# ideafisher/ssUnet-GAN

Measured on AMD Instinct MI355X. Metric: train images/sec (512^2 tiles), higher is better.
Workload: dtype f32; 1 GPU; UNet_R_SS_v2 generator + SRGAN-style discriminator, one G+D step (train_seg_gan.py:182-233), 16 x 3x512x512 tiles per GPU, fp32, Adam lr 2e-5; global_batch=16, tile=512, parallelism=dp1, dead_d_param_grads_of_g_step=computed

## Files before the change

### include/ssunet_hip.h

```cpp
#ifndef SSUNET_HIP_H
#define SSUNET_HIP_H

#include <stdint.h>

#ifdef __cplusplus
extern "C" {
#endif

#define SSG_OK 0
#define SSG_EINVAL (-1)
#define SSG_EALIGN (-2)

#define SSG_ACT_NONE 0
#define SSG_ACT_RELU 1
#define SSG_ACT_LRELU 2
#define SSG_ACT_SWISH 3

#define SSG_MAX_TAPS 9

const char* ssg_last_error(void);
int ssg_abi_version(void);

typedef struct {
  const float* in1; const float* in2;
// ... 154 lines not shown
                        float* mean, float* invstd, float* scale, float* shift, void* stream);

typedef struct ssg_bn_fin {
  const float* weight; const float* bias;
  float eps, momentum; int var_mode;
  float* running_mean; float* running_var;
  float* mean; float* invstd; float* scale; float* shift;
} ssg_bn_fin;
int ssg_bn_stats_finalize_f32(const float* x, int64_t P, int C, int ld, const ssg_bn_fin* fin, void* ws, void* stream);
int ssg_bn_stats_finalize_bf16(const void* x, int64_t P, int C, int ld, const ssg_bn_fin* fin, void* ws, void* stream);
int ssg_bn_stats_from_partials_finalize_f32(const double* part, int rows, int C, double count, const ssg_bn_fin* fin, void* ws, void* stream);
int ssg_bn_apply_f32(const float* x, int64_t P, int C, int ld, const float* scale, const float* shift,
                     const float* res, int ldr, int act, float slope, float* y, int ldy, void* stream);
int ssg_bn_bwd_reduce_f32(const float* x, const float* y, const float* dy, int64_t P, int C,
                          int ldx, int ldy, int lddy, const float* mean, const float* invstd,
                          const float* scale, const float* shift,
                          int act, float slope, double* sums, int with_count, void* ws, void* stream);
int ssg_bn_bwd_apply_f32(const float* x, const float* y, const float* dy, int64_t P, int C,
                         int ldx, int ldy, int lddy, const float* mean, const float* invstd,
                         const float* weight, const float* scale, const float* shift,
                         const double* sums, double count, int act, float slope,
                         float* dx, int lddx, float* dres, int lddres,
                         float* dweight, float* dbias, void* stream);
int ssg_bn_frozen_bwd_f32(const float* x, const float* y, const float* dy, int64_t P, int C, int ldx, int ldy, int lddy,
                          const float* mean, const float* invstd, const float* scale, const float* shift, int act, float slope,
                          float* dx, int lddx, float* dres, int lddres, double* sums, void* ws, void* stream);
int ssg_bn_fold_bwd_f32(const float* dwf, const float* w, int Cout, int64_t K, const float* s, const float* mean,
                        const float* invstd, const double* sums_g, float* dw, float* dgamma, float* dbeta, void* stream);

int ssg_maxpool2x2_fwd_f32(const float* x, int N, int H, int W, int C, int ldx, float* y, int ldy, uint8_t* idx, void* stream);
int ssg_maxpool2x2_bwd_f32(const float* dy, int lddy, const uint8_t* idx, int N, int H, int W, int C, float* dx, int lddx, void* stream);
int ssg_maxpool2x2_bwd_add_f32(const float* dy, int lddy, const uint8_t* idx, const float* res, int ldr, int N, int H, int W, int C,
                               float* dx, int lddx, void* stream);
int ssg_maxunpool2x2_fwd_f32(const float* x, int ldx, const uint8_t* idx, int N, int OH, int OW, int C, float* y, int ldy, void* stream);
int ssg_maxunpool2x2_bwd_f32(const float* dy, int lddy, const uint8_t* idx, int N, int OH, int OW, int C, float* dx, int lddx, void* stream);
int ssg_upsample2x_bilinear_fwd_f32(const float* x, int N, int H, int W, int C, int ldx, float* y, int ldy, void* stream);
int ssg_upsample2x_bilinear_bwd_f32(const float* dy, int lddy, int N, int H, int W, int C, float* dx, int lddx, void* stream);
int ssg_upsample2x_nearest_fwd_f32(const float* x, int N, int H, int W, int C, int ldx, float* y, int ldy, void* stream);
int ssg_upsample2x_nearest_bwd_f32(const float* dy, int lddy, int N, int H, int W, int C, float* dx, int lddx, void* stream);
int ssg_adaptive_avgpool_flat_fwd_f32(const float* x, int N, int H, int W, int C, int ldx, int OHW, float* y, void* stream);
int ssg_adaptive_avgpool_flat_bwd_f32(const float* dy, int N, int H, int W, int C, int OHW, float* dx, int lddx, void* stream);

int ssg_spade_conv_modulate_ok(const ssg_conv_desc* d);
int ssg_spade_conv_modulate_f32(const ssg_conv_desc* d, const float* x, int ldx, float* gamma, int ldg, void* stream);
int ssg_spade_modulate_fwd_f32(const float* x, int ldx, const float* gb, int ldgb, int64_t P, int C, float* y, int ldy, void* stream);
int ssg_spade_modulate_bwd_f32(const float* x, int ldx, const float* gb, int ldgb, const float* dy, int lddy, int64_t P, int C,
// ... 97 lines not shown
```

### ssunet-gan_amd/_lib.py

```python
import ctypes as C
import os

import torch

_HERE = os.path.dirname(os.path.abspath(__file__))
LIB_PATH = os.environ.get('SSG_LIB_PATH') or os.path.join(_HERE, 'libssunet_hip.so')
MAX_TAPS = 9
ACT_NONE, ACT_RELU, ACT_LRELU, ACT_SWISH = 0, 1, 2, 3


class HipLibraryError(RuntimeError):
    pass


class ConvDesc(C.Structure):
    _fields_ = [
        ('in1', C.c_void_p), ('in2', C.c_void_p),
        ('C1', C.c_int), ('C2', C.c_int), ('ld1', C.c_int), ('ld2', C.c_int),
        ('N', C.c_int), ('H', C.c_int), ('W', C.c_int),
        ('w', C.c_void_p), ('Kp', C.c_int), ('kmode', C.c_int),
        ('bias', C.c_void_p),
        ('res', C.c_void_p), ('ldr', C.c_int),
        ('out', C.c_void_p), ('Cout', C.c_int), ('ldo', C.c_int),
        ('GH', C.c_int), ('GW', C.c_int), ('OH', C.c_int), ('OW', C.c_int),
# ... 80 lines not shown
    'ssg_conv2d_wgrad_bf16x2_ok': [C.POINTER(WgradDesc)],
    'ssg_conv2d_wgrad_bf16x2_kernel_id': [C.POINTER(WgradDesc)],
    'ssg_conv2d_wgrad_bf16x2_workspace_bytes': [C.POINTER(WgradDesc)],
    'ssg_conv2d_wgrad_bf16x2_f32': [C.POINTER(WgradDesc), _P],
    'ssg_conv2d_wgrad_bf16x1_s2_ok': [C.POINTER(WgradDesc)],
    'ssg_conv2d_wgrad_bf16x1_s2_kernel_id': [C.POINTER(WgradDesc)],
    'ssg_conv2d_wgrad_bf16x1_s2_workspace_bytes': [C.POINTER(WgradDesc)],
    'ssg_conv2d_wgrad_bf16x1_s2_f32': [C.POINTER(WgradDesc), _P],
    'ssg_bn_stats_from_partials_workspace_bytes': [_I, _I],
    'ssg_bn_stats_from_partials_f32': [_P, _I, _I, _P, _D, _P, _P],
    'ssg_conv2d_wgrad_kernel_id': [C.POINTER(WgradDesc)],
    'ssg_pack_weights_f32': [_P, _I, _I, _I, _I, _I, _I, C.POINTER(C.c_int), C.POINTER(C.c_int), _I, _I, _I, _P, _P],
    'ssg_pack_weights_scaled_f32': [_P, _I, _I, _I, _I, _I, _I, C.POINTER(C.c_int), C.POINTER(C.c_int), _I, _I, _I, _P, _P, _P],
    'ssg_conv2d_wgrad_workspace_bytes': [C.POINTER(WgradDesc)],
    'ssg_conv2d_wgrad_f32': [C.POINTER(WgradDesc), _P],
    'ssg_nchw_to_nhwc_f32': [_P, _I, _I, _I, _I, _P, _I, _P],
    'ssg_nhwc_to_nchw_f32': [_P, _I, _I, _I, _I, _I, _P, _P],
    'ssg_bn_workspace_bytes': [_L, _I],
    'ssg_bn_stats_f32': [_P, _L, _I, _I, _P, _I, _P, _P],
    'ssg_bn_finalize_f32': [_P, _D, _I, _P, _P, _F, _F, _I, _P, _P, _P, _P, _P, _P, _P],
    'ssg_bn_apply_f32': [_P, _L, _I, _I, _P, _P, _P, _I, _I, _F, _P, _I, _P],
    'ssg_bn_bwd_reduce_f32': [_P, _P, _P, _L, _I, _I, _I, _I, _P, _P, _P, _P, _I, _F, _P, _I, _P, _P],
    'ssg_bn_bwd_apply_f32': [_P, _P, _P, _L, _I, _I, _I, _I, _P, _P, _P, _P, _P, _P, _D, _I, _F, _P, _I, _P, _I, _P, _P, _P],
    'ssg_bn_frozen_bwd_f32': [_P, _P, _P, _L, _I, _I, _I, _I, _P, _P, _P, _P, _I, _F, _P, _I, _P, _I, _P, _P, _P],
    'ssg_bn_fold_bwd_f32': [_P, _P, _I, _L, _P, _P, _P, _P, _P, _P, _P, _P],
    'ssg_maxpool2x2_fwd_f32': [_P, _I, _I, _I, _I, _I, _P, _I, _P, _P],
    'ssg_maxpool2x2_bwd_f32': [_P, _I, _P, _I, _I, _I, _I, _P, _I, _P],
    'ssg_maxpool2x2_bwd_add_f32': [_P, _I, _P, _P, _I, _I, _I, _I, _I, _P, _I, _P],
    'ssg_maxunpool2x2_fwd_f32': [_P, _I, _P, _I, _I, _I, _I, _P, _I, _P],
    'ssg_maxunpool2x2_bwd_f32': [_P, _I, _P, _I, _I, _I, _I, _P, _I, _P],
    'ssg_upsample2x_bilinear_fwd_f32': [_P, _I, _I, _I, _I, _I, _P, _I, _P],
    'ssg_upsample2x_bilinear_bwd_f32': [_P, _I, _I, _I, _I, _I, _P, _I, _P],
    'ssg_upsample2x_nearest_fwd_f32': [_P, _I, _I, _I, _I, _I, _P, _I, _P],
    'ssg_upsample2x_nearest_bwd_f32': [_P, _I, _I, _I, _I, _I, _P, _I, _P],
    'ssg_adaptive_avgpool_flat_fwd_f32': [_P, _I, _I, _I, _I, _I, _I, _P, _P],
    'ssg_adaptive_avgpool_flat_bwd_f32': [_P, _I, _I, _I, _I, _I, _P, _I, _P],
    'ssg_spade_conv_modulate_ok': [C.POINTER(ConvDesc)],
    'ssg_spade_conv_modulate_f32': [C.POINTER(ConvDesc), _P, _I, _P, _I, _P],
    'ssg_spade_modulate_fwd_f32': [_P, _I, _P, _I, _L, _I, _P, _I, _P],
    'ssg_spade_modulate_bwd_f32': [_P, _I, _P, _I, _P, _I, _L, _I, _P, _I, _P, _I, _P],
    'ssg_spade_modulate_bwd_sums_f32': [_P, _I, _P, _I, _P, _I, _L, _I, _P, _I, _P, _I, _P, _P, _P],
    'ssg_act_bwd_f32': [_P, _I, _P, _I, _L, _I, _I, _F, _P, _I, _P],
    'ssg_add_f32': [_P, _P, _L, _P, _P],
    'ssg_copy_channels_f32': [_P, _I, _L, _I, _P, _I, _P],
    'ssg_nan_to_zero_f32': [_P, _L, _P, _P],
    'ssg_mask_zero_f32': [_P, _P, _L, _P, _P],
# ... 139 lines not shown
```

### ssunet-gan_amd/blocks.py

```python
import ctypes as C
import os

import torch

from . import ops
from ._lib import ACT_NONE, ACT_RELU, call, ptr, stream_ptr
from .ops import (_act_bwd, _bn_bwd_impl, _bn_fwd_impl, _channel_sum, _conv_dgrad_impl, _conv_fwd_impl, _conv_wgrad_impl,
                  _ld, new_nhwc, to_nhwc)


def _x_mode(stride):
    mode = ops.train_precision_mode()
    return mode if mode != 'fp32' and stride == 1 else False


class _BasicBlockFn(torch.autograd.Function):

    @staticmethod
    def forward(ctx, x1, x2, w1, g1, b1, rm1, rv1, w2, g2, b2, rm2, rv2, wsc, eps1, mom1, eps2, mom2, stride, var_mode, group):
        x1 = to_nhwc(x1)
        x2 = to_nhwc(x2) if x2 is not None else None
        ctx.x1m = x1m = _x_mode(stride)
        p3 = x1m or 'fp32'
        c1, part1 = _conv_fwd_impl(x1, x2, w1, None, stride, 1, ACT_NONE, 0.0, want_bn=True, precision=p3)
# ... 55 lines not shown
        dx1 = dx2 = None
        if stride != 1 and (need_x1 or need_x2):
            raise NotImplementedError('strided BasicBlock input gradient')
        if need_x1:
            part = _conv_dgrad_impl(g, wsc, 1, 0, h, w, 0, ca) if wsc is not None else g
            dx1 = _conv_dgrad_impl(dc1, w1, 1, 1, h, w, 0, ca, res=part, precision=p3)
        if need_x2:
            part = _conv_dgrad_impl(g, wsc, 1, 0, h, w, ca, ca + cb)
            dx2 = _conv_dgrad_impl(dc1, w1, 1, 1, h, w, ca, ca + cb, res=part, precision=p3)
        return (dx1, dx2, dw1, dg1, db1, None, None, dw2, dg2, db2, None, None, dwsc,
                None, None, None, None, None, None, None)


def basic_block(x1, x2, conv1, bn1, conv2, bn2, shortcut_conv, group=None):
    for bn in (bn1, bn2):
        if bn.track_running_stats and bn.num_batches_tracked is not None and not ops._synced(group):
            bn.num_batches_tracked.add_(1)
    var_mode = getattr(bn1, '_ssg_var_mode', 1 if group is not None else 0)
    return _BasicBlockFn.apply(x1, x2, conv1.weight, bn1.weight, bn1.bias, bn1.running_mean, bn1.running_var,
                               conv2.weight, bn2.weight, bn2.bias, bn2.running_mean, bn2.running_var,
                               shortcut_conv.weight if shortcut_conv is not None else None,
                               float(bn1.eps), float(bn1.momentum), float(bn2.eps), float(bn2.momentum),
                               int(conv1.stride[0]), var_mode, group)


def _fold_bwd(dwf, w, s, mean, invstd, sums_g, need_w, need_gb):
    o = w.shape[0]
    dw = torch.empty_like(dwf) if need_w else None
    dgb = torch.empty((2, o), dtype=torch.float32, device=w.device) if need_gb else None
    wc = w.detach().contiguous()
    call('ssg_bn_fold_bwd_f32', ptr(dwf), ptr(wc), o, wc.numel() // o, ptr(s), ptr(mean), ptr(invstd), ptr(sums_g), ptr(dw),
         ptr(dgb[0]) if need_gb else None, ptr(dgb[1]) if need_gb else None, stream_ptr())
    return dw, (dgb[0] if need_gb else None), (dgb[1] if need_gb else None)


class _FrozenBasicBlockFn(torch.autograd.Function):

    @staticmethod
    def forward(ctx, x1, x2, w1, g1, b1, w2, g2, b2, wsc, wf1, bf1, wf2, bf2, k1, k2, stride, record):
        x1 = to_nhwc(x1)
        x2 = to_nhwc(x2) if x2 is not None else None
        x1m = record and any(ctx.needs_input_grad) and _x_mode(stride)
        p3 = x1m or 'fp32'
        y1 = _conv_fwd_impl(x1, x2, wf1, bf1, stride, 1, ACT_RELU, 0.0, precision=p3)
        if wsc is not None:
            r = _conv_fwd_impl(x1, x2, wsc, None, stride, 0, ACT_NONE, 0.0)
# ... 233 lines not shown
```

### ssunet-gan_amd/csrc/bn.hip

```cpp
#include "common.h"

namespace {

constexpr int RED_BLOCK = 256;
constexpr int MAX_PARTS = 1024;

struct RedGeom { int TQ, PR, groups, parts; long long rows_per_part; };

__host__ RedGeom red_geom(long long P, int C, int Q = 1) {
  RedGeom g;
  const int CQ = (C + 4 * Q - 1) / (4 * Q);
  g.TQ = CQ >= 64 ? 64 : 1;
  if (CQ < 64) { while (g.TQ < CQ) g.TQ <<= 1; }
  g.PR = RED_BLOCK / g.TQ;
  g.groups = (CQ + g.TQ - 1) / g.TQ;
  long long parts = (P + (long long)g.PR * 8 - 1) / ((long long)g.PR * 8);
  if (parts > MAX_PARTS) parts = MAX_PARTS;
  if (parts < 1) parts = 1;
  g.rows_per_part = (P + parts - 1) / parts;
  g.parts = (int)((P + g.rows_per_part - 1) / g.rows_per_part);
  return g;
}

template <int MODE, typename T>
// ... 252 lines not shown
                                                       const T* __restrict__ res, int ldr, int act, float slope,
                                                       T* __restrict__ y, int ldy) {
  constexpr int Q = SsgQ<T>::value;
  const int CG = C / (4 * Q);
  const long long total = P * CG;
  SSG_CHUNK_LOOP(i, total) {
    const long long p = i / CG; const int c0 = 4 * Q * (int)(i - p * CG);
    f32x4 xv[Q], rv[Q], o[Q];
    ldq(x + p * ld + c0, xv);
    if (res) ldq(res + p * ldr + c0, rv);
#pragma unroll
    for (int q = 0; q < Q; ++q) {
      const f32x4 sc = *(const f32x4*)(scale + c0 + 4 * q), sh = *(const f32x4*)(shift + c0 + 4 * q);
      f32x4 v = xv[q] * sc + sh;
      if (res) v += rv[q];
#pragma unroll
      for (int e = 0; e < 4; ++e) v[e] = ssg_act(v[e], act, slope);
      o[q] = v;
    }
    stq(y + p * ldy + c0, o);
  }
}

template <typename T>
__global__ __launch_bounds__(256) void bn_bwd_apply_kernel(
    const T* __restrict__ x, const T* __restrict__ y, const T* __restrict__ dy, long long P, int C, int ldx,
    int ldy, int lddy, const float* __restrict__ mean, const float* __restrict__ invstd, const float* __restrict__ weight,
    const float* __restrict__ scale, const float* __restrict__ shift,
    const double* __restrict__ sums, double count_arg, int act, float slope, T* __restrict__ dx, int lddx,
    T* __restrict__ dres, int lddres, float* __restrict__ dweight, float* __restrict__ dbias) {
  const double count = count_arg > 0 ? count_arg : sums[2 * C];
  if (blockIdx.x == 0) {
    for (int c = threadIdx.x; c < C; c += 256) {
      if (dweight) dweight[c] = (float)sums[C + c];
      if (dbias) dbias[c] = (float)sums[c];
    }
  }
  typedef typename SsgAcc<T>::type acc_t;
  extern __shared__ double kc_raw[];
  acc_t* kc = (acc_t*)kc_raw;
  acc_t* k_mean = kc; acc_t* k_is = kc + C; acc_t* k_ws = kc + 2 * C; acc_t* k_m1 = kc + 3 * C; acc_t* k_m2 = kc + 4 * C;
  for (int c = threadIdx.x; c < C; c += 256) {
    const double is = (double)invstd[c];
    k_mean[c] = (acc_t)mean[c]; k_is[c] = (acc_t)is; k_ws[c] = (acc_t)((weight ? (double)weight[c] : 1.0) * is);
    k_m1[c] = (acc_t)(sums[c] / count); k_m2[c] = (acc_t)(sums[C + c] / count);
  }
  __syncthreads();
  constexpr int Q = SsgQ<T>::value;
  const int CG = C / (4 * Q);
  const long long totalg = P * CG;
  SSG_CHUNK_LOOP(i, totalg) {
    const long long p = i / CG; const int c0 = 4 * Q * (int)(i - p * CG);
    f32x4 gq[Q], xq[Q], yq[Q], oq[Q];
    ldq(dy + p * lddy + c0, gq);
    ldq(x + p * ldx + c0, xq);
    const bool use_y = act != SSG_ACT_NONE && act != SSG_ACT_SWISH && y;
    if (use_y) ldq(y + p * ldy + c0, yq);
#pragma unroll
    for (int q = 0; q < Q; ++q) {
      const int cb = c0 + 4 * q;
      f32x4 g = gq[q];
      const f32x4 xv = xq[q];
      if (act == SSG_ACT_SWISH) {
        const f32x4 z = xv * *(const f32x4*)(scale + cb) + *(const f32x4*)(shift + cb);
#pragma unroll
        for (int e = 0; e < 4; ++e) g[e] *= ssg_swish_grad(z[e]);
      } else if (act != SSG_ACT_NONE) {
        const f32x4 yv = use_y ? yq[q] : xv * *(const f32x4*)(scale + cb) + *(const f32x4*)(shift + cb);
#pragma unroll
        for (int e = 0; e < 4; ++e) if (!(yv[e] > 0.f)) g[e] *= (act == SSG_ACT_RELU ? 0.f : slope);
      }
      gq[q] = g;
      if (dx) {
        f32x4 o;
#pragma unroll
        for (int e = 0; e < 4; ++e) {
          const int c = cb + e;
          const acc_t xh = ((acc_t)xv[e] - k_mean[c]) * k_is[c];
          o[e] = (float)(k_ws[c] * ((acc_t)g[e] - k_m1[c] - xh * k_m2[c]));
        }
        oq[q] = o;
      }
    }
    if (dres) stq(dres + p * lddres + c0, gq);
    if (dx) stq(dx + p * lddx + c0, oq);
  }
}

int elem_grid(long long total) { return ssg_elem_grid(total, 4); }

template <int MODE, typename T>
int run_reduce(const T* x, const T* y, const T* dy, long long P, int C, int ldx, int ldy, int lddy,
               const float* scale, const float* shift,
               const float* mean, const float* invstd, int act, float slope, double* sums, float* fsum, void* ws,
               hipStream_t st, double count_out = 0.0, BnFin fin = BnFin{}, double fin_count = 0.0) {
  constexpr int Q = SsgQ<T>::value;
  const RedGeom g = red_geom(P, C, Q);
  const int C4 = 4 * Q * ((C + 4 * Q - 1) / (4 * Q));
  double* part = (double*)ws;
  hipLaunchKernelGGL((col_reduce_kernel<MODE, T>), dim3((unsigned)g.parts, (unsigned)g.groups), dim3(RED_BLOCK), 0, st, x, y, dy,
                     P, C, ldx, ldy, lddy, mean, invstd, scale, shift, act, slope, g.TQ, g.PR, g.rows_per_part, part, (T*)nullptr, 0, (T*)nullptr, 0);
  SSG_LAUNCH_CHECK();
  hipLaunchKernelGGL(col_reduce_final_kernel, dim3((unsigned)((C + 31) / 32)), dim3(32 * FIN_LANES), 0, st, part, g.parts, C, C4, sums, fsum, count_out, fin, fin_count);
  SSG_LAUNCH_CHECK();
  return SSG_OK;
}

}
// ... 26 lines not shown
  SSG_REQUIRE(!(act == SSG_ACT_SWISH && res), SSG_EINVAL, "bn_apply: swish with a residual is not supported (its backward needs the pre-activation)");
  hipLaunchKernelGGL(bn_apply_kernel<T>, dim3((unsigned)elem_grid(P * (C / (4 * SsgQ<T>::value)))), dim3(256), 0, (hipStream_t)stream, x, (long long)P, C, ld,
                     scale, shift, res, ldr, act, slope, y, ldy);
  SSG_LAUNCH_CHECK();
  return SSG_OK;
}

template <typename T>
int bn_bwd_reduce_impl(const T* x, const T* y, const T* dy, int64_t P, int C, int ldx, int ldy, int lddy, const float* mean,
                       const float* invstd, const float* scale, const float* shift, int act, float slope, double* sums, int with_count,
                       void* ws, void* stream) {
  SSG_REQUIRE(x && dy && mean && invstd && sums && ws && P > 0 && C > 0, SSG_EINVAL, "bn_bwd_reduce: bad args");
  SSG_REQUIRE(act == SSG_ACT_NONE || (y && act != SSG_ACT_SWISH) || (scale && shift), SSG_EINVAL,
              "bn_bwd_reduce: activation gradient needs y (ReLU family only) or (scale, shift)");
  SSG_REQUIRE(C % (4 * SsgQ<T>::value) == 0 && ldx % (4 * SsgQ<T>::value) == 0 && lddy % (4 * SsgQ<T>::value) == 0 && ssg_aligned16(x) && ssg_aligned16(dy),
              SSG_EALIGN, "bn_bwd_reduce: C / ld must be multiples of 4 (fp32) or 8 (bf16), rows 16-byte aligned");
  return run_reduce<1, T>(x, y, dy, P, C, ldx, ldy, lddy, scale, shift, mean, invstd, act, slope, sums, nullptr, ws, (hipStream_t)stream,
                          with_count ? (double)P : 0.0);
}

template <typename T>
int bn_bwd_apply_impl(const T* x, const T* y, const T* dy, int64_t P, int C, int ldx, int ldy, int lddy, const float* mean,
                      const float* invstd, const float* weight, const float* scale, const float* shift, const double* sums, double count,
                      int act, float slope, T* dx, int lddx, T* dres, int lddres, float* dweight, float* dbias, void* stream) {
  SSG_REQUIRE(x && dy && mean && invstd && sums && P > 0 && C > 0, SSG_EINVAL, "bn_bwd_apply: bad args");
  SSG_REQUIRE(act == SSG_ACT_NONE || (y && act != SSG_ACT_SWISH) || (scale && shift), SSG_EINVAL,
              "bn_bwd_apply: activation gradient needs y (ReLU family only) or (scale, shift)");
  constexpr int G = 4 * SsgQ<T>::value;
  SSG_REQUIRE(C % G == 0 && ldx % G == 0 && lddy % G == 0 && (!y || ldy % G == 0) && (!dx || lddx % G == 0) && (!dres || lddres % G == 0) &&
                  ssg_aligned16(x) && ssg_aligned16(dy) && (!dx || ssg_aligned16(dx)), SSG_EALIGN,
              "bn_bwd_apply: C/ld must be multiples of 4 (fp32) or 8 (bf16), rows 16-byte aligned");
  SSG_REQUIRE(C <= 4096, SSG_EINVAL, "bn_bwd_apply: C > 4096");
  if ((size_t)5 * C * sizeof(double) > 48 * 1024) {
    hipError_t e = hipFuncSetAttribute((const void*)bn_bwd_apply_kernel<T>, hipFuncAttributeMaxDynamicSharedMemorySize, 5 * C * (int)sizeof(double));
    if (e != hipSuccess) { ssg_set_error("bn_bwd_apply: LDS attribute: %s", hipGetErrorString(e)); return (int)e; }
  }
  hipLaunchKernelGGL(bn_bwd_apply_kernel<T>, dim3((unsigned)elem_grid(P * (C / (4 * SsgQ<T>::value)))), dim3(256), (size_t)5 * C * sizeof(double), (hipStream_t)stream, x, y, dy,
                     (long long)P, C, ldx, ldy, lddy, mean, invstd, weight, scale, shift, sums, count, act, slope, dx, lddx, dres, lddres,
                     dweight, dbias);
  SSG_LAUNCH_CHECK();
  return SSG_OK;
}

}

extern "C" int ssg_bn_stats_f32(const float* x, int64_t P, int C, int ld, double* sums, int with_count, void* ws, void* stream) {
  return bn_stats_impl<float>(x, P, C, ld, sums, with_count, ws, stream);
}
extern "C" int ssg_bn_stats_bf16(const void* x, int64_t P, int C, int ld, double* sums, int with_count, void* ws, void* stream) {
  return bn_stats_impl<ssg_bf16>((const ssg_bf16*)x, P, C, ld, sums, with_count, ws, stream);
}

namespace {
constexpr int FOLD_Z = 64;
__global__ __launch_bounds__(256) void bnpart_fold_kernel(const double* __restrict__ part, int rows, int C, int rows_per_z,
                                                          double* __restrict__ out ) {
  __shared__ double red[2][8][32];
  const int cl = threadIdx.x & 31, rl = threadIdx.x >> 5;
  const int c = blockIdx.x * 32 + cl;
  const int r0 = blockIdx.y * rows_per_z;
  int r1 = r0 + rows_per_z; if (r1 > rows) r1 = rows;
  double a1 = 0, a2 = 0;
// ... 92 lines not shown
                                 const void* res, int ldr, int act, float slope, void* y, int ldy, void* stream) {
  return bn_apply_impl<ssg_bf16>((const ssg_bf16*)x, P, C, ld, scale, shift, (const ssg_bf16*)res, ldr, act, slope, (ssg_bf16*)y, ldy, stream);
}

extern "C" int ssg_bn_bwd_reduce_f32(const float* x, const float* y, const float* dy, int64_t P, int C, int ldx, int ldy,
                                     int lddy, const float* mean, const float* invstd, const float* scale, const float* shift,
                                     int act, float slope, double* sums, int with_count, void* ws, void* stream) {
  return bn_bwd_reduce_impl<float>(x, y, dy, P, C, ldx, ldy, lddy, mean, invstd, scale, shift, act, slope, sums, with_count, ws, stream);
}
extern "C" int ssg_bn_bwd_reduce_bf16(const void* x, const void* y, const void* dy, int64_t P, int C, int ldx, int ldy,
                                      int lddy, const float* mean, const float* invstd, const float* scale, const float* shift,
                                      int act, float slope, double* sums, int with_count, void* ws, void* stream) {
  return bn_bwd_reduce_impl<ssg_bf16>((const ssg_bf16*)x, (const ssg_bf16*)y, (const ssg_bf16*)dy, P, C, ldx, ldy, lddy, mean, invstd, scale, shift,
                                      act, slope, sums, with_count, ws, stream);
}

extern "C" int ssg_bn_bwd_apply_f32(const float* x, const float* y, const float* dy, int64_t P, int C, int ldx, int ldy,
                                    int lddy, const float* mean, const float* invstd, const float* weight,
                                    const float* scale, const float* shift, const double* sums,
                                    double count, int act, float slope, float* dx, int lddx, float* dres, int lddres,
                                    float* dweight, float* dbias, void* stream) {
  return bn_bwd_apply_impl<float>(x, y, dy, P, C, ldx, ldy, lddy, mean, invstd, weight, scale, shift, sums, count, act, slope, dx, lddx, dres,
                                  lddres, dweight, dbias, stream);
}
extern "C" int ssg_bn_bwd_apply_bf16(const void* x, const void* y, const void* dy, int64_t P, int C, int ldx, int ldy,
                                     int lddy, const float* mean, const float* invstd, const float* weight,
                                     const float* scale, const float* shift, const double* sums,
                                     double count, int act, float slope, void* dx, int lddx, void* dres, int lddres,
                                     float* dweight, float* dbias, void* stream) {
  return bn_bwd_apply_impl<ssg_bf16>((const ssg_bf16*)x, (const ssg_bf16*)y, (const ssg_bf16*)dy, P, C, ldx, ldy, lddy, mean, invstd, weight, scale,
                                     shift, sums, count, act, slope, (ssg_bf16*)dx, lddx, (ssg_bf16*)dres, lddres, dweight, dbias, stream);
}

extern "C" int ssg_spade_modulate_bwd_sums_f32(const float* x, int ldx, const float* gb, int ldgb, const float* dy, int lddy, int64_t P,
                                               int C, float* dx, int lddx, float* dgb, int lddgb, double* sums, void* ws, void* stream) {
  SSG_REQUIRE(x && gb && dy && dx && dgb && sums && ws && P > 0 && C > 0 && C % 4 == 0 && ldgb >= C && lddgb >= 2 * C, SSG_EINVAL,
              "modulate_bwd_sums: bad args");
  const RedGeom g = red_geom(P, C);
  double* part = (double*)ws;
  hipStream_t st = (hipStream_t)stream;
  hipLaunchKernelGGL(modulate_bwd_sums_kernel, dim3((unsigned)g.parts, (unsigned)g.groups), dim3(RED_BLOCK), 0, st, x, ldx, gb, ldgb, dy, lddy,
                     (long long)P, C, dx, lddx, dgb, lddgb, g.TQ, g.PR, g.rows_per_part, part);
  SSG_LAUNCH_CHECK();
  hipLaunchKernelGGL(col_reduce_final_kernel, dim3((unsigned)((C + 31) / 32)), dim3(32 * FIN_LANES), 0, st, part, g.parts, C, C, sums, nullptr, 0.0, BnFin{}, 0.0);
  SSG_LAUNCH_CHECK();
  return SSG_OK;
// ... 88 lines not shown
```

### ssunet-gan_amd/models_seg_gan.py

```python
import os

import torch
import torch.nn as nn

from . import archs, ops
from ._lib import ACT_LRELU, ACT_NONE
from .spectral_norm import SpectralNorm


def remove_prefix(state_dict, prefix):
    f = lambda x: x.split(prefix, 1)[-1] if x.startswith(prefix) else x
    return {f(key): value for key, value in state_dict.items()}


class ConvolutionalBlock(nn.Module):

    def __init__(self, in_channels, out_channels, kernel_size, stride=1, batch_norm=False, activation=None):
        super().__init__()
        if activation is not None:
            activation = activation.lower()
            assert activation in {'prelu', 'leakyrelu', 'tanh'}
        layers = [nn.Conv2d(in_channels=in_channels, out_channels=out_channels, kernel_size=kernel_size, stride=stride,
                            padding=kernel_size // 2)]
        if batch_norm is True:
            layers.append(nn.BatchNorm2d(num_features=out_channels))
        if activation == 'prelu':
            layers.append(nn.PReLU())
        elif activation == 'leakyrelu':
# ... 10 lines not shown
        for hook in conv._forward_pre_hooks.values():
            if isinstance(hook, SpectralNorm) and hook.name == 'weight' and hook.dim == 0 and conv.weight_orig.is_cuda:
                sn = hook
            else:
                hook(conv, (input,))
        if self._act not in (None, 'leakyrelu'):
            raise NotImplementedError('ConvolutionalBlock activation %r has no HIP path (only the discriminator\'s '
                                      'LeakyReLU flavour is on the hot path)' % self._act)
        act = ACT_LRELU if self._act == 'leakyrelu' else ACT_NONE
        slope = self.conv_block[-1].negative_slope if act == ACT_LRELU else 0.0
        if sn is not None:
            def run(a, sl):
                return ops.conv2d_sn(input, conv.weight_orig, conv.weight_u, conv.weight_v, conv.bias, conv.stride[0], conv.padding[0],
                                     act=a, slope=sl, n_power_iterations=sn.n_power_iterations if conv.training else 0, eps=sn.eps)
        else:
            precision, wgrad_s2 = ops.train_precision_mode(), ops.train_wgrad_s2_mode()

            def run(a, sl, bn_stats=False):
                return ops.conv2d(input, conv.weight, conv.bias, conv.stride[0], conv.padding[0], act=a, slope=sl, bn_stats=bn_stats,
                                  precision=precision, wgrad_s2=wgrad_s2)
        if not self._bn:
            return run(act, slope)
        bn = self.conv_block[1]
        part = None
        if sn is None and bn.training:
            y, part = run(ACT_NONE, 0.0, bn_stats=True)
        else:
            y = run(ACT_NONE, 0.0)
        return ops.batch_norm_act(y, bn, act=act, slope=slope, group=getattr(bn, '_ssg_sync_group', None), stats_part=part)


class Generator(nn.Module):

    def __init__(self, config):
        super().__init__()
        if config['arch'] not in archs.__all__:
            raise NotImplementedError('arch %r is not built in ssunet-gan_amd (available: %s)' % (config['arch'], archs.__all__))
        self.net = archs.__dict__[config['arch']](config['num_classes'], config['input_channels'], config['deep_supervision'])

    def initialize_with_srresnet(self, model_folder, config):
        model_dict = torch.load(os.path.join(model_folder, '%s/model.pth' % config['name']), map_location='cpu')
        if 'state_dict' in model_dict.keys():
            model_dict = remove_prefix(model_dict['state_dict'], 'module.')
        else:
            model_dict = remove_prefix(model_dict, 'module.')
        missing, unexpected = self.net.load_state_dict(model_dict, strict=False)
        if missing or unexpected:
            raise RuntimeError('checkpoint key mismatch: missing %s unexpected %s' % (missing[:5], unexpected[:5]))
        print("\nLoaded weights from pre-trained SS-UNet-R.\n")

    def forward(self, lr_imgs):
        return self.net(lr_imgs)
# ... 26 lines not shown
```

### ssunet-gan_amd/ops.py

```python
import ctypes as C
import math

import torch
import torch.distributed as dist

from . import _lib
from ._lib import ACT_LRELU, ACT_NONE, ACT_RELU, ACT_SWISH, ConvDesc, WgradDesc, call, ptr, stream_ptr

__all__ = ['conv2d', 'batch_norm_act', 'max_pool2x2', 'max_pool2x2_skip', 'max_unpool2x2', 'upsample2x_bilinear', 'upsample2x_nearest',
           'spade_modulate', 'adaptive_avgpool_flat', 'linear', 'seg_loss', 'bce_with_logits_const', 'nan_to_zero_',
           'to_nhwc', 'new_nhwc', 'bump_weight_epoch', 'dwconv2d', 'swish', 'sigmoid', 'gaussian', 'mul', 'global_avgpool',
           'channel_scale', 'spectral_norm_weight', 'conv2d_sn']


def pad4(c):
    return (c + 3) // 4 * 4


def new_nhwc(n, c, h, w, device, ld=None, zero=False):
    ld = pad4(c) if ld is None else ld
    buf = (torch.zeros if zero else torch.empty)(n * h * w * ld, device=device, dtype=torch.float32)
    return torch.empty(0, device=device, dtype=torch.float32).set_(
        buf.untyped_storage(), 0, (n, c, h, w), (h * w * ld, 1, w * ld, ld))

# ... 505 lines not shown
        ctx.set_materialize_grads(False)
        x1 = to_nhwc(x1)
        x2 = to_nhwc(x2) if x2 is not None else None
        res = to_nhwc(res) if res is not None else None
        r = _conv_fwd_impl(x1, x2, weight, bias, stride, pad, act, slope, res=res, want_bn=want_bn, precision=precision, x1_s2=True)
        y, part = r if want_bn else (r, None)
        ctx.cfg = (stride, pad, act, slope, precision, wgrad_s2)
        ctx.save_for_backward(x1, x2, weight, y if act != ACT_NONE else None)
        ctx.has_bias = bias is not None
        ctx.has_res = res is not None
        if part is None:
            part = torch.empty(0, dtype=torch.float64, device=y.device)
        ctx.mark_non_differentiable(part)
        return y, part

    @staticmethod
    @torch.autograd.function.once_differentiable
    def backward(ctx, dy, _=None):
        if dy is None:
            return (None,) * 12
        x1, x2, weight, y = ctx.saved_tensors
        stride, pad, act, slope, precision, wgrad_s2 = ctx.cfg
        dy = to_nhwc(dy)
        if act != ACT_NONE:
            dy = _act_bwd(y, dy, act, slope)
        n, c1, h, w = x1.shape
        dx1 = dx2 = dw = db = None
        if ctx.needs_input_grad[0]:
            dx1 = _conv_dgrad_impl(dy, weight, stride, pad, h, w, 0, c1, precision=precision, x1_s2=True)
        if x2 is not None and ctx.needs_input_grad[1]:
            dx2 = _conv_dgrad_impl(dy, weight, stride, pad, h, w, c1, c1 + x2.shape[1], precision=precision, x1_s2=True)
        if ctx.needs_input_grad[2]:
            dw = _conv_wgrad_impl(x1, x2, dy, weight.shape, stride, pad, precision=precision, wgrad_s2=wgrad_s2)
        if ctx.has_bias and ctx.needs_input_grad[3]:
            db = _channel_sum(dy, weight.shape[0])
        dres = dy if (ctx.has_res and ctx.needs_input_grad[8]) else None
        return dx1, dx2, dw, db, None, None, None, None, dres, None, None, None


def conv2d(x, weight, bias=None, stride=1, padding=0, act=ACT_NONE, slope=0.0, x2=None, res=None, bn_stats=False, precision='fp32',
           wgrad_s2='fp32'):
    _lib.require_gpu(x)
    if precision not in _PRECISIONS:
        raise ValueError('conv2d: unknown precision %r (one of %s)' % (precision, ', '.join(_PRECISIONS)))
    _check_wgrad_s2('conv2d', precision, wgrad_s2)
    pad = tuple(int(v) for v in padding) if isinstance(padding, (tuple, list)) else int(padding)
    y, part = _Conv2d.apply(x, x2, weight, bias, int(stride), pad, int(act), float(slope), res, bool(bn_stats), precision, wgrad_s2)
    return (y, part) if bn_stats else y


_X1_LABELS = {70: 'conv_halo_k32_x1_kernel<128>', 71: 'conv_halo_k32_x1_kernel<64>'}
_X1_KIND = (_X1_LABELS, 'ssg_conv2d_bf16x1_kernel_id', _CONV_SHAPE)
_X1_TAPS = _taps_fwd(3, 3, 1)
_PRECISIONS = ('fp32', 'bf16x1', 'bf16x2')
_X2_LABELS = {90: 'conv_halo_k32_x2_kernel<128>', 91: 'conv_halo_k32_x2_kernel<64>'}
_X2_KIND = (_X2_LABELS, 'ssg_conv2d_bf16x2_kernel_id', _CONV_SHAPE)
_WGRAD_X2_LABELS = {92: 'wgrad_k32_x2_kernel'}
# ... 431 lines not shown
        else:
            ws = _ws(call('ssg_bn_workspace_bytes', p, c), dev)
            call('ssg_bn_stats_finalize_f32', ptr(x), p, c, _ld(x), C.byref(fin), ptr(ws), stream_ptr())
        sums = None
    else:
        sums = torch.empty(2 * c + 1, dtype=torch.float64, device=dev)
        if have_part:
            rows = part.numel() // (2 * c)
            ws = _ws(call('ssg_bn_stats_from_partials_workspace_bytes', rows, c), dev)
            call('ssg_bn_stats_from_partials_f32', ptr(part), rows, c, ptr(sums), float(p) if synced else 0.0, ptr(ws), stream_ptr())
        else:
            ws = _ws(call('ssg_bn_workspace_bytes', p, c), dev)
            call('ssg_bn_stats_f32', ptr(x), p, c, _ld(x), ptr(sums), int(synced), ptr(ws), stream_ptr())
        if synced:
            _timed_all_reduce('sync_bn_fwd', sums, group)
        call('ssg_bn_finalize_f32', ptr(sums), 0.0 if synced else float(p), c, ptr(weight), ptr(bias), eps, momentum, var_mode,
             ptr(running_mean), ptr(running_var), ptr(stats[0]), ptr(stats[1]), ptr(stats[2]), ptr(stats[3]), stream_ptr())
    if running_mean is not None or running_var is not None:
        _STATS_EPOCH[0] += 1
    y = _bn_apply(x, stats, res, act, slope) if apply else None
    return y, stats, (sums[2 * c:] if synced else None)


def _bn_bwd_impl(x, y, dy, weight, stats, act, slope, group, count, want_dres, want_dx=True, had_res=True):
    n, c, h, w = x.shape
    with _hbm('bn_bwd', 4.0 * n * h * w * c * (3 + (1 if want_dx else 0) + (1 if want_dres else 0))):
        return _bn_bwd_body(x, y, dy, weight, stats, act, slope, group, count, want_dres, want_dx, had_res)


def _bn_bwd_body(x, y, dy, weight, stats, act, slope, group, count, want_dres, want_dx=True, had_res=True):
    n, c, h, w = x.shape
    p = n * h * w
    dev = x.device
    if act == ACT_NONE or not had_res:
        y = None
    synced = count is not None
    ws = _ws(call('ssg_bn_workspace_bytes', p, c), dev)
    sums = torch.empty(2 * c + 1, dtype=torch.float64, device=dev)
    call('ssg_bn_bwd_reduce_f32', ptr(x), ptr(y), ptr(dy), p, c, _ld(x), _ld(y) if y is not None else 0, _ld(dy),
         ptr(stats[0]), ptr(stats[1]), ptr(stats[2]), ptr(stats[3]), act, slope, ptr(sums), int(synced), ptr(ws), stream_ptr())
    local = sums.clone() if synced else sums
    if synced:
        _timed_all_reduce('sync_bn_bwd', sums, group)
    dwb = torch.empty((2, c), dtype=torch.float32, device=dev)
    dx = new_nhwc(n, c, h, w, dev) if want_dx else None
    dres = new_nhwc(n, c, h, w, dev) if want_dres else None
    call('ssg_bn_bwd_apply_f32', ptr(x), ptr(y), ptr(dy), p, c, _ld(x), _ld(y) if y is not None else 0, _ld(dy),
         ptr(stats[0]), ptr(stats[1]), ptr(weight), ptr(stats[2]), ptr(stats[3]), ptr(sums), 0.0 if synced else float(p), act, slope,
         ptr(dx), _ld(dx) if dx is not None else 0, ptr(dres), _ld(dres) if dres is not None else 0,
         ptr(dwb[0]), ptr(dwb[1]), stream_ptr())
    if synced:
        dwb = torch.stack([local[c:2 * c], local[:c]]).float()
    return dx, dres, dwb[0], dwb[1]


BN_BWD_EPILOGUE = _os.environ.get('SSG_BN_BWD_EPILOGUE', '0') == '1'


def _bn_bwd_from_partials(x, g, part, weight, stats, group, count):
    n, c, h, w = x.shape
    p = n * h * w
    dev = x.device
    synced = count is not None
    rows = part.numel() // (2 * c)
    sums = torch.empty(2 * c + 1, dtype=torch.float64, device=dev)
    ws = _ws(call('ssg_bn_stats_from_partials_workspace_bytes', rows, c), dev)
    call('ssg_bn_stats_from_partials_f32', ptr(part), rows, c, ptr(sums), float(p) if synced else 0.0, ptr(ws), stream_ptr())
    sums[c:2 * c] *= stats[1].double()
    local = sums.clone() if synced else sums
    if synced:
        _timed_all_reduce('sync_bn_bwd', sums, group)
    dwb = torch.empty((2, c), dtype=torch.float32, device=dev)
    dx = new_nhwc(n, c, h, w, dev)
    with _hbm('bn_bwd', 4.0 * p * c * 3):
        call('ssg_bn_bwd_apply_f32', ptr(x), None, ptr(g), p, c, _ld(x), 0, _ld(g),
# ... 1031 lines not shown
```

Before: 91.04 images/sec.

## Fuse conv bias gradient into BN backward apply and activation backward

Adds a fused conv+BN+act autograd function whose backward computes the conv bias gradient as per-channel sums of dx inside the BN backward apply kernel. This uses a partitioned reduction layout plus a final column reduce. The plain conv backward also takes the bias sum from the frozen activation-backward reduction instead of a separate channel-sum pass. The goal is to remove extra full-tensor reads for the bias gradient, at the cost of a different grid shape for the apply kernel and an extra small reduce launch.

```diff
diff --git a/include/ssunet_hip.h b/include/ssunet_hip.h
--- a/include/ssunet_hip.h
+++ b/include/ssunet_hip.h
@@ -200,6 +200,12 @@
                          const double* sums, double count, int act, float slope,
                          float* dx, int lddx, float* dres, int lddres,
                          float* dweight, float* dbias, void* stream);
+int ssg_bn_bwd_apply_sums_f32(const float* x, const float* y, const float* dy, int64_t P, int C,
+                              int ldx, int ldy, int lddy, const float* mean, const float* invstd,
+                              const float* weight, const float* scale, const float* shift,
+                              const double* sums, double count, int act, float slope,
+                              float* dx, int lddx, float* dres, int lddres,
+                              float* dweight, float* dbias, double* dx_sums, float* dx_fsums, void* ws, void* stream);
 int ssg_bn_frozen_bwd_f32(const float* x, const float* y, const float* dy, int64_t P, int C, int ldx, int ldy, int lddy,
                           const float* mean, const float* invstd, const float* scale, const float* shift, int act, float slope,
                           float* dx, int lddx, float* dres, int lddres, double* sums, void* ws, void* stream);
diff --git a/ssunet-gan_amd/_lib.py b/ssunet-gan_amd/_lib.py
--- a/ssunet-gan_amd/_lib.py
+++ b/ssunet-gan_amd/_lib.py
@@ -126,6 +126,7 @@
     'ssg_bn_apply_f32': [_P, _L, _I, _I, _P, _P, _P, _I, _I, _F, _P, _I, _P],
     'ssg_bn_bwd_reduce_f32': [_P, _P, _P, _L, _I, _I, _I, _I, _P, _P, _P, _P, _I, _F, _P, _I, _P, _P],
     'ssg_bn_bwd_apply_f32': [_P, _P, _P, _L, _I, _I, _I, _I, _P, _P, _P, _P, _P, _P, _D, _I, _F, _P, _I, _P, _I, _P, _P, _P],
+    'ssg_bn_bwd_apply_sums_f32': [_P, _P, _P, _L, _I, _I, _I, _I, _P, _P, _P, _P, _P, _P, _D, _I, _F, _P, _I, _P, _I, _P, _P, _P, _P, _P, _P],
     'ssg_bn_frozen_bwd_f32': [_P, _P, _P, _L, _I, _I, _I, _I, _P, _P, _P, _P, _I, _F, _P, _I, _P, _I, _P, _P, _P],
     'ssg_bn_fold_bwd_f32': [_P, _P, _I, _L, _P, _P, _P, _P, _P, _P, _P, _P],
     'ssg_maxpool2x2_fwd_f32': [_P, _I, _I, _I, _I, _I, _P, _I, _P, _P],
diff --git a/ssunet-gan_amd/blocks.py b/ssunet-gan_amd/blocks.py
--- a/ssunet-gan_amd/blocks.py
+++ b/ssunet-gan_amd/blocks.py
@@ -101,6 +101,47 @@
                                shortcut_conv.weight if shortcut_conv is not None else None,
                                float(bn1.eps), float(bn1.momentum), float(bn2.eps), float(bn2.momentum),
                                int(conv1.stride[0]), var_mode, group)
+
+
+class _ConvBnActFn(torch.autograd.Function):
+
+    @staticmethod
+    def forward(ctx, x, w, bias, g, b, rm, rv, stride, pad, eps, mom, act, slope, var_mode, group, precision, wgrad_s2):
+        x = to_nhwc(x)
+        c, part = _conv_fwd_impl(x, None, w, bias, stride, pad, ACT_NONE, 0.0, want_bn=True, precision=precision, x1_s2=True)
+        y, st, cnt = _bn_fwd_impl(c, g, b, rm, rv, None, eps, mom, act, slope, var_mode, group, part=part)
+        ctx.save_for_backward(x, c, w, g, st)
+        ctx.cfg = (stride, pad, act, slope, group, cnt, precision, wgrad_s2)
+        return y
+
+    @staticmethod
+    @torch.autograd.function.once_differentiable
+    def backward(ctx, dy):
+        x, c, w, g, st = ctx.saved_tensors
+        stride, pad, act, slope, group, cnt, precision, wgrad_s2 = ctx.cfg
+        dy = to_nhwc(dy)
+        dc, _, dg, dbeta, dbias = _bn_bwd_impl(c, None, dy, g, st, act, slope, group, cnt, want_dres=False, had_res=False, dx_sums=True)
+        dx = dw = None
+        if ctx.needs_input_grad[0]:
+            dx = _conv_dgrad_impl(dc, w, stride, pad, x.shape[2], x.shape[3], 0, x.shape[1], precision=precision, x1_s2=True)
+        if ctx.needs_input_grad[1]:
+            dw = _conv_wgrad_impl(x, None, dc, w.shape, stride, pad, precision=precision, wgrad_s2=wgrad_s2)
+        return (dx, dw, dbias if ctx.needs_input_grad[2] else None, dg, dbeta) + (None,) * 12
+
+
+def conv_bn_act(x, conv, bn, act, slope, group=None, precision='fp32', wgrad_s2='fp32'):
+    ops._lib.require_gpu(x)
+    if precision not in ops._PRECISIONS:
+        raise ValueError('conv_bn_act: unknown precision %r (one of %s)' % (precision, ', '.join(ops._PRECISIONS)))
+    ops._check_wgrad_s2('conv_bn_act', precision, wgrad_s2)
+    if bn.momentum is None:
+        raise NotImplementedError('cumulative-average batch norm (momentum=None)')
+    if bn.track_running_stats and bn.num_batches_tracked is not None and not ops._synced(group):
+        bn.num_batches_tracked.add_(1)
+    var_mode = getattr(bn, '_ssg_var_mode', 1 if group is not None else 0)
+    return _ConvBnActFn.apply(x, conv.weight, conv.bias, bn.weight, bn.bias, bn.running_mean if bn.track_running_stats else None,
+                              bn.running_var if bn.track_running_stats else None, int(conv.stride[0]), int(conv.padding[0]),
+                              float(bn.eps), float(bn.momentum), int(act), float(slope), int(var_mode), group, precision, wgrad_s2)
 
 
 def _fold_bwd(dwf, w, s, mean, invstd, sums_g, need_w, need_gb):
diff --git a/ssunet-gan_amd/csrc/bn.hip b/ssunet-gan_amd/csrc/bn.hip
--- a/ssunet-gan_amd/csrc/bn.hip
+++ b/ssunet-gan_amd/csrc/bn.hip
@@ -298,15 +298,16 @@
   }
 }
 
-template <typename T>
+template <typename T, bool DXSUMS = false>
 __global__ __launch_bounds__(256) void bn_bwd_apply_kernel(
     const T* __restrict__ x, const T* __restrict__ y, const T* __restrict__ dy, long long P, int C, int ldx,
     int ldy, int lddy, const float* __restrict__ mean, const float* __restrict__ invstd, const float* __restrict__ weight,
     const float* __restrict__ scale, const float* __restrict__ shift,
     const double* __restrict__ sums, double count_arg, int act, float slope, T* __restrict__ dx, int lddx,
-    T* __restrict__ dres, int lddres, float* __restrict__ dweight, float* __restrict__ dbias) {
+    T* __restrict__ dres, int lddres, float* __restrict__ dweight, float* __restrict__ dbias,
+    int TQ, int PR, long long rows_per_part, double* __restrict__ part) {
   const double count = count_arg > 0 ? count_arg : sums[2 * C];
-  if (blockIdx.x == 0) {
+  if (blockIdx.x == 0 && (!DXSUMS || blockIdx.y == 0)) {
     for (int c = threadIdx.x; c < C; c += 256) {
       if (dweight) dweight[c] = (float)sums[C + c];
       if (dbias) dbias[c] = (float)sums[c];
@@ -325,8 +326,25 @@
   constexpr int Q = SsgQ<T>::value;
   const int CG = C / (4 * Q);
   const long long totalg = P * CG;
-  SSG_CHUNK_LOOP(i, totalg) {
-    const long long p = i / CG; const int c0 = 4 * Q * (int)(i - p * CG);
+  static_assert(!DXSUMS || Q == 1, "the dx sums add the fp32 values as stored: fp32 tensors only");
+  long long it, it_end, it_step;
+  int c_own = 0, tq = 0, pr = 0;
+  double acc[4 * Q];
+#pragma unroll
+  for (int e = 0; e < 4 * Q; ++e) acc[e] = 0;
+  if constexpr (DXSUMS) {
+    tq = threadIdx.x % TQ; pr = threadIdx.x / TQ;
+    const int cg = blockIdx.y * TQ + tq;
+    c_own = cg < CG ? 4 * Q * cg : -1;
+    const long long p0 = (long long)blockIdx.x * rows_per_part;
+    long long p1 = p0 + rows_per_part; if (p1 > P) p1 = P;
+    it = c_own >= 0 ? p0 + pr : p1; it_end = p1; it_step = PR;
+  } else {
+    it = ssg_chunk_begin(totalg) + threadIdx.x; it_end = ssg_chunk_end(totalg); it_step = 256;
+  }
+  for (long long i = it; i < it_end; i += it_step) {
+    long long p; int c0;
+    if constexpr (DXSUMS) { p = i; c0 = c_own; } else { p = i / CG; c0 = 4 * Q * (int)(i - p * CG); }
     f32x4 gq[Q], xq[Q], yq[Q], oq[Q];
     ldq(dy + p * lddy + c0, gq);
     ldq(x + p * ldx + c0, xq);
@@ -354,12 +372,30 @@
           const int c = cb + e;
           const acc_t xh = ((acc_t)xv[e] - k_mean[c]) * k_is[c];
           o[e] = (float)(k_ws[c] * ((acc_t)g[e] - k_m1[c] - xh * k_m2[c]));
+          if constexpr (DXSUMS) acc[4 * q + e] += (double)o[e];
         }
         oq[q] = o;
       }
     }
     if (dres) stq(dres + p * lddres + c0, gq);
     if (dx) stq(dx + p * lddx + c0, oq);
+  }
+  if constexpr (DXSUMS) {
+    __shared__ double red[RED_BLOCK][4 * Q];
+#pragma unroll
+    for (int e = 0; e < 4 * Q; ++e) red[threadIdx.x][e] = acc[e];
+    __syncthreads();
+    if (pr == 0 && c_own >= 0) {
+      double a[4 * Q];
+#pragma unroll
+      for (int e = 0; e < 4 * Q; ++e) a[e] = 0;
+      for (int r = 0; r < PR; ++r)
+#pragma unroll
+        for (int e = 0; e < 4 * Q; ++e) a[e] += red[r * TQ + tq][e];
+      double* dst = part + (size_t)blockIdx.x * 2 * C;
+#pragma unroll
+      for (int e = 0; e < 4 * Q; ++e) { dst[c_own + e] = a[e]; dst[C + c_own + e] = 0.0; }
+    }
   }
 }
 
@@ -432,8 +468,11 @@
 template <typename T>
 int bn_bwd_apply_impl(const T* x, const T* y, const T* dy, int64_t P, int C, int ldx, int ldy, int lddy, const float* mean,
                       const float* invstd, const float* weight, const float* scale, const float* shift, const double* sums, double count,
-                      int act, float slope, T* dx, int lddx, T* dres, int lddres, float* dweight, float* dbias, void* stream) {
+                      int act, float slope, T* dx, int lddx, T* dres, int lddres, float* dweight, float* dbias, void* stream,
+                      double* dx_sums = nullptr, float* dx_fsums = nullptr, void* ws = nullptr) {
   SSG_REQUIRE(x && dy && mean && invstd && sums && P > 0 && C > 0, SSG_EINVAL, "bn_bwd_apply: bad args");
+  const bool want_sums = dx_sums || dx_fsums;
+  SSG_REQUIRE(!want_sums || (dx && ws && SsgQ<T>::value == 1), SSG_EINVAL, "bn_bwd_apply: dx sums need dx, a workspace and fp32 tensors");
   SSG_REQUIRE(act == SSG_ACT_NONE || (y && act != SSG_ACT_SWISH) || (scale && shift), SSG_EINVAL,
               "bn_bwd_apply: activation gradient needs y (ReLU family only) or (scale, shift)");
   constexpr int G = 4 * SsgQ<T>::value;
@@ -441,13 +480,32 @@
                   ssg_aligned16(x) && ssg_aligned16(dy) && (!dx || ssg_aligned16(dx)), SSG_EALIGN,
               "bn_bwd_apply: C/ld must be multiples of 4 (fp32) or 8 (bf16), rows 16-byte aligned");
   SSG_REQUIRE(C <= 4096, SSG_EINVAL, "bn_bwd_apply: C > 4096");
+  if constexpr (SsgQ<T>::value == 1) {
+    if (want_sums) {
+      SSG_REQUIRE(C <= 3840, SSG_EINVAL, "bn_bwd_apply: dx sums need C <= 3840");
+      if ((size_t)5 * C * sizeof(double) > 40 * 1024) {
+        hipError_t e = hipFuncSetAttribute((const void*)bn_bwd_apply_kernel<T, true>, hipFuncAttributeMaxDynamicSharedMemorySize, 5 * C * (int)sizeof(double));
+        if (e != hipSuccess) { ssg_set_error("bn_bwd_apply: LDS attribute: %s", hipGetErrorString(e)); return (int)e; }
+      }
+      const RedGeom g = red_geom(P, C, 1);
+      hipStream_t st = (hipStream_t)stream;
+      hipLaunchKernelGGL((bn_bwd_apply_kernel<T, true>), dim3((unsigned)g.parts, (unsigned)g.groups), dim3(256), (size_t)5 * C * sizeof(double), st, x, y, dy,
+                         (long long)P, C, ldx, ldy, lddy, mean, invstd, weight, scale, shift, sums, count, act, slope, dx, lddx, dres, lddres,
+                         dweight, dbias, g.TQ, g.PR, g.rows_per_part, (double*)ws);
+      SSG_LAUNCH_CHECK();
+      hipLaunchKernelGGL(col_reduce_final_kernel, dim3((unsigned)((C + 31) / 32)), dim3(32 * FIN_LANES), 0, st, (const double*)ws, g.parts, C, C, dx_sums,
+                         dx_fsums, 0.0, BnFin{}, 0.0);
+      SSG_LAUNCH_CHECK();
+      return SSG_OK;
+    }
+  }
   if ((size_t)5 * C * sizeof(double) > 48 * 1024) {
     hipError_t e = hipFuncSetAttribute((const void*)bn_bwd_apply_kernel<T>, hipFuncAttributeMaxDynamicSharedMemorySize, 5 * C * (int)sizeof(double));
     if (e != hipSuccess) { ssg_set_error("bn_bwd_apply: LDS attribute: %s", hipGetErrorString(e)); return (int)e; }
   }
   hipLaunchKernelGGL(bn_bwd_apply_kernel<T>, dim3((unsigned)elem_grid(P * (C / (4 * SsgQ<T>::value)))), dim3(256), (size_t)5 * C * sizeof(double), (hipStream_t)stream, x, y, dy,
                      (long long)P, C, ldx, ldy, lddy, mean, invstd, weight, scale, shift, sums, count, act, slope, dx, lddx, dres, lddres,
-                     dweight, dbias);
+                     dweight, dbias, 0, 0, 0ll, (double*)nullptr);
   SSG_LAUNCH_CHECK();
   return SSG_OK;
 }
@@ -586,6 +644,15 @@
                                     float* dweight, float* dbias, void* stream) {
   return bn_bwd_apply_impl<float>(x, y, dy, P, C, ldx, ldy, lddy, mean, invstd, weight, scale, shift, sums, count, act, slope, dx, lddx, dres,
                                   lddres, dweight, dbias, stream);
+}
+extern "C" int ssg_bn_bwd_apply_sums_f32(const float* x, const float* y, const float* dy, int64_t P, int C, int ldx, int ldy,
+                                         int lddy, const float* mean, const float* invstd, const float* weight,
+                                         const float* scale, const float* shift, const double* sums,
+                                         double count, int act, float slope, float* dx, int lddx, float* dres, int lddres,
+                                         float* dweight, float* dbias, double* dx_sums, float* dx_fsums, void* ws, void* stream) {
+  SSG_REQUIRE(dx && (dx_sums || dx_fsums) && ws, SSG_EINVAL, "bn_bwd_apply_sums: dx, one of dx_sums / dx_fsums and the workspace are required");
+  return bn_bwd_apply_impl<float>(x, y, dy, P, C, ldx, ldy, lddy, mean, invstd, weight, scale, shift, sums, count, act, slope, dx, lddx, dres,
+                                  lddres, dweight, dbias, stream, dx_sums, dx_fsums, ws);
 }
 extern "C" int ssg_bn_bwd_apply_bf16(const void* x, const void* y, const void* dy, int64_t P, int C, int ldx, int ldy,
                                      int lddy, const float* mean, const float* invstd, const float* weight,
diff --git a/ssunet-gan_amd/models_seg_gan.py b/ssunet-gan_amd/models_seg_gan.py
--- a/ssunet-gan_amd/models_seg_gan.py
+++ b/ssunet-gan_amd/models_seg_gan.py
@@ -3,7 +3,7 @@
 import torch
 import torch.nn as nn
 
-from . import archs, ops
+from . import archs, blocks, ops
 from ._lib import ACT_LRELU, ACT_NONE
 from .spectral_norm import SpectralNorm
 
@@ -60,12 +60,16 @@
         if not self._bn:
             return run(act, slope)
         bn = self.conv_block[1]
+        group = getattr(bn, '_ssg_sync_group', None)
+        if (ops.BIAS_FOLD and sn is None and bn.training and conv.bias is not None and bn.weight is not None
+                and conv.out_channels % 4 == 0):
+            return blocks.conv_bn_act(input, conv, bn, act, slope, group=group, precision=precision, wgrad_s2=wgrad_s2)
         part = None
         if sn is None and bn.training:
             y, part = run(ACT_NONE, 0.0, bn_stats=True)
         else:
             y = run(ACT_NONE, 0.0)
-        return ops.batch_norm_act(y, bn, act=act, slope=slope, group=getattr(bn, '_ssg_sync_group', None), stats_part=part)
+        return ops.batch_norm_act(y, bn, act=act, slope=slope, group=group, stats_part=part)
 
 
 class Generator(nn.Module):
diff --git a/ssunet-gan_amd/ops.py b/ssunet-gan_amd/ops.py
--- a/ssunet-gan_amd/ops.py
+++ b/ssunet-gan_amd/ops.py
@@ -551,17 +551,21 @@
         x1, x2, weight, y = ctx.saved_tensors
         stride, pad, act, slope, precision, wgrad_s2 = ctx.cfg
         dy = to_nhwc(dy)
-        if act != ACT_NONE:
+        dx1 = dx2 = dw = db = None
+        want_db = ctx.has_bias and ctx.needs_input_grad[3]
+        if BIAS_FOLD and want_db and act in (ACT_RELU, ACT_LRELU) and dy.shape[1] % 4 == 0:
+            dy, _, sums = _frozen_bwd(None, y, dy, None, None, None, None, act, slope)
+            db = sums[:dy.shape[1]].float()
+        elif act != ACT_NONE:
             dy = _act_bwd(y, dy, act, slope)
         n, c1, h, w = x1.shape
-        dx1 = dx2 = dw = db = None
         if ctx.needs_input_grad[0]:
             dx1 = _conv_dgrad_impl(dy, weight, stride, pad, h, w, 0, c1, precision=precision, x1_s2=True)
         if x2 is not None and ctx.needs_input_grad[1]:
             dx2 = _conv_dgrad_impl(dy, weight, stride, pad, h, w, c1, c1 + x2.shape[1], precision=precision, x1_s2=True)
         if ctx.needs_input_grad[2]:
             dw = _conv_wgrad_impl(x1, x2, dy, weight.shape, stride, pad, precision=precision, wgrad_s2=wgrad_s2)
-        if ctx.has_bias and ctx.needs_input_grad[3]:
+        if want_db and db is None:
             db = _channel_sum(dy, weight.shape[0])
         dres = dy if (ctx.has_res and ctx.needs_input_grad[8]) else None
         return dx1, dx2, dw, db, None, None, None, None, dres, None, None, None
@@ -1039,13 +1043,16 @@
     return y, stats, (sums[2 * c:] if synced else None)
 
 
-def _bn_bwd_impl(x, y, dy, weight, stats, act, slope, group, count, want_dres, want_dx=True, had_res=True):
+def _bn_bwd_impl(x, y, dy, weight, stats, act, slope, group, count, want_dres, want_dx=True, had_res=True, dx_sums=False):
     n, c, h, w = x.shape
     with _hbm('bn_bwd', 4.0 * n * h * w * c * (3 + (1 if want_dx else 0) + (1 if want_dres else 0))):
-        return _bn_bwd_body(x, y, dy, weight, stats, act, slope, group, count, want_dres, want_dx, had_res)
-
-
-def _bn_bwd_body(x, y, dy, weight, stats, act, slope, group, count, want_dres, want_dx=True, had_res=True):
+        return _bn_bwd_body(x, y, dy, weight, stats, act, slope, group, count, want_dres, want_dx, had_res, dx_sums)
+
+
+BIAS_FOLD = _os.environ.get('SSG_BIAS_FOLD', '1') != '0'
+
+
+def _bn_bwd_body(x, y, dy, weight, stats, act, slope, group, count, want_dres, want_dx=True, had_res=True, dx_sums=False):
     n, c, h, w = x.shape
     p = n * h * w
     dev = x.device
@@ -1062,12 +1069,19 @@
     dwb = torch.empty((2, c), dtype=torch.float32, device=dev)
     dx = new_nhwc(n, c, h, w, dev) if want_dx else None
     dres = new_nhwc(n, c, h, w, dev) if want_dres else None
-    call('ssg_bn_bwd_apply_f32', ptr(x), ptr(y), ptr(dy), p, c, _ld(x), _ld(y) if y is not None else 0, _ld(dy),
-         ptr(stats[0]), ptr(stats[1]), ptr(weight), ptr(stats[2]), ptr(stats[3]), ptr(sums), 0.0 if synced else float(p), act, slope,
-         ptr(dx), _ld(dx) if dx is not None else 0, ptr(dres), _ld(dres) if dres is not None else 0,
-         ptr(dwb[0]), ptr(dwb[1]), stream_ptr())
+    args = (ptr(x), ptr(y), ptr(dy), p, c, _ld(x), _ld(y) if y is not None else 0, _ld(dy),
+            ptr(stats[0]), ptr(stats[1]), ptr(weight), ptr(stats[2]), ptr(stats[3]), ptr(sums), 0.0 if synced else float(p), act, slope,
+            ptr(dx), _ld(dx) if dx is not None else 0, ptr(dres), _ld(dres) if dres is not None else 0,
+            ptr(dwb[0]), ptr(dwb[1]))
+    if dx_sums:
+        dxs = torch.empty(c, dtype=torch.float32, device=dev)
+        call('ssg_bn_bwd_apply_sums_f32', *args, None, ptr(dxs), ptr(ws), stream_ptr())
+    else:
+        call('ssg_bn_bwd_apply_f32', *args, stream_ptr())
     if synced:
         dwb = torch.stack([local[c:2 * c], local[:c]]).float()
+    if dx_sums:
+        return dx, dres, dwb[0], dwb[1], dxs
     return dx, dres, dwb[0], dwb[1]
 
 
```

Result: no change. 91.33 images/sec, median of 3 (+0.3%).
